# gorjanradevski/revisiting-spatial-temporal-layouts

Hardware: AMD Instinct MI355X
Metric: clips/s STLT forward (T=32, N_obj=7, d=768) (higher is better)
Workload: dtype f32; 1 GPU; cfg2: STLT forward, T=32, N=7, d=768, H=12, 4+8 layers, 174 classes; per_gpu_batch=1024, global_batch=1024, parallelism=batch-shard x1, no collective, cls_only_last_spatial=True

## Files before the change

include/stlt_hip.h:

```cpp
#ifndef STLT_HIP_H
#define STLT_HIP_H

#include <stddef.h>
#include <stdint.h>

#ifdef __cplusplus
extern "C" {
#endif

#define STLT_VERSION 110

#define STLT_EINVAL (-1)
#define STLT_EWORKSPACE (-2)

#define STLT_ACT_NONE 0
#define STLT_ACT_GELU 1
#define STLT_ACT_RELU 2

typedef void* stlt_stream_t;

int stlt_version(void);
const char* stlt_last_error(void);

typedef struct stlt_ctx stlt_ctx;
// ... 5 lines not shown
                   const float* box_w, const float* box_b, const float* score_w, const float* score_b,
                   const float* ln_w, const float* ln_b, float eps,
                   int64_t n_tokens, int64_t d, float* out, stlt_stream_t stream);

int stlt_linear_fwd(const float* x, int64_t ldx, const float* w, const float* bias,
                    float* y, int64_t ldy, int64_t M, int64_t N, int64_t K, int act, stlt_stream_t stream);

int stlt_gemm(int transA, int transB, const float* a, int64_t lda, const float* b, int64_t ldb,
              const float* r, int64_t ldr, float* c, int64_t ldc, int64_t slab_stride,
              int64_t M, int64_t N, int64_t K, int n_split, stlt_stream_t stream);
int stlt_linear_small_fwd(const float* x, int64_t ldx, const float* w, const float* bias, const float* r, int64_t ldr, float* y, int64_t ldy,
                          int64_t M, int64_t N, int64_t K, int act, int tile, stlt_stream_t stream);
int stlt_linear_small_choice(int64_t M, int64_t N, int64_t K);
int stlt_input_grad_small(const float* dy, int64_t ld_dy, const float* w, int64_t n_out, int64_t k_in, const float* r, int64_t ldr, float* dx,
                          int64_t ld_dx, int64_t M, int tile, stlt_ctx* ctx, stlt_stream_t stream);
int stlt_input_grad_small_choice(int64_t M, int64_t n_out, int64_t k_in);
int stlt_set_gemm_small_tiles(int mode);

size_t stlt_gemm_scratch_bytes(void);
int stlt_gemm_set_scratch(void* scratch, size_t bytes);
typedef struct { const float* dy; int64_t n_out; const float* x; int64_t k_in; int64_t rows; float* g_w; } stlt_wgrad_item;
int stlt_weight_grad_group(const stlt_wgrad_item* items, int n_items, stlt_stream_t stream);
int stlt_reduce_slabs(const float* slabs, int64_t stride, int n_slabs, float* dst, int64_t n, int accumulate,
                      stlt_stream_t stream);

int stlt_attn_core_fwd(const float* qkv, const uint8_t* kpm, int causal,
                       int64_t S, int64_t L, int64_t H, int64_t dh, float* ctx, stlt_stream_t stream);

int stlt_mhsa_fused_fwd(const float* x, const float* in_proj_w, const float* in_proj_b, const uint8_t* kpm, int64_t S, int64_t L,
                        int64_t H, int64_t d, float* ctx, stlt_stream_t stream);
int stlt_mhsa_fused_fwd_ex(const float* x, const float* in_proj_w, const float* in_proj_b, const uint8_t* kpm, int causal, int64_t S,
                           int64_t L, int64_t H, int64_t d, float dropout_p, uint64_t seed, uint32_t site, float* ctx, float* qkv_out,
                           stlt_stream_t stream);
int stlt_fused_mhsa_active(int64_t T, int64_t d, int64_t H);
int stlt_fused_mhsa_used(int64_t S, int64_t L, int64_t d, int64_t H, int causal);
int stlt_attn_cross_fwd(const float* q, int64_t ldq, const float* k, const float* v, int64_t ldkv, const uint8_t* kpm,
                        int causal, int64_t S, int64_t Lq, int64_t Lk, int64_t H, int64_t dh, float* ctx,
                        stlt_stream_t stream);

int stlt_attn_ragged_fwd(const float* qkv, const int32_t* seg_start, const int32_t* seg_end, int causal, int64_t M,
                         int64_t H, int64_t dh, float* ctx, stlt_stream_t stream);

int stlt_add_layernorm_fwd(const float* x, int64_t ldx, const float* res, int64_t ldres,
                           const float* ln_w, const float* ln_b, float eps,
                           int64_t M, int64_t d, float* out, int64_t ldout, stlt_stream_t stream);

int stlt_frames_embed_fwd(const float* spatial, int64_t row_stride, const int64_t* frame_types,
                          const float* pos_table, const float* type_table,
                          const float* ln_w, const float* ln_b, float eps,
                          int64_t B, int64_t T, int64_t d, float* out, stlt_stream_t stream);

int stlt_gather_last_fwd(const float* x, const int64_t* lengths, int64_t B, int64_t T, int64_t d,
                         float* out, stlt_stream_t stream);

int stlt_collate_fwd(const int64_t* categories_ragged, const float* boxes_ragged, const float* scores_ragged,
                     const int64_t* frame_types_ragged, const int64_t* frame_offsets, int64_t B, int64_t T, int64_t N,
                     int64_t cls_id, int64_t* categories, float* boxes, float* scores, int64_t* frame_types,
                     uint8_t* kpm_boxes, uint8_t* kpm_frames, stlt_stream_t stream);

typedef struct {
  int64_t src_offset;
  int32_t h, w;
  int32_t rh, rw;
  int32_t top, left;
  int32_t tab_x, ksize_x;
  int32_t tab_y, ksize_y;
// ... 308 lines not shown
```

revisiting-spatial-temporal-layouts_amd/_lib.py:

```python
from __future__ import annotations

import ctypes as C
import os

HERE = os.path.dirname(os.path.abspath(__file__))
LIB_PATH = os.environ.get("STLT_HIP_LIB") or os.path.join(HERE, "libstlt_hip.so")

K_NAMES = ("embed", "gemm", "attn_spatial", "attn_temporal", "add_layernorm", "frames_embed", "gather_last", "ln_bwd", "attn_bwd",
           "gelu", "embed_bwd", "optim", "misc", "mhsa_fused", "mhsa_fused_spatial")
FLAG_CLS_ONLY_LAST_SPATIAL = 1
FLAG_LAST_ROW_ONLY_TEMPORAL = 2
FLAG_SKIP_PADDING = 4
FLAG_TRAIN_UPPER_ONLY = 8
FLAG_TRAIN_LOWER_ONLY = 16
FLAG_TRAIN_BACKBONE = 32
ACT_NONE, ACT_GELU, ACT_RELU = 0, 1, 2

_f = C.POINTER(C.c_float)
_i64 = C.POINTER(C.c_int64)
_u8 = C.POINTER(C.c_uint8)
_vp = C.c_void_p


class OptChunk(C.Structure):
# ... 103 lines not shown
    "stlt_version": (C.c_int, []),
    "stlt_last_error": (C.c_char_p, []),
    "stlt_embed_fwd": (C.c_int, [_vp, _vp, _vp, _vp, C.c_int64, _vp, _vp, _vp, _vp, _vp, _vp, C.c_float,
                                 C.c_int64, C.c_int64, _vp, _vp]),
    "stlt_linear_fwd": (C.c_int, [_vp, C.c_int64, _vp, _vp, _vp, C.c_int64, C.c_int64, C.c_int64, C.c_int64,
                                  C.c_int, _vp]),
    "stlt_linear_small_fwd": (C.c_int, [_vp, C.c_int64, _vp, _vp, _vp, C.c_int64, _vp, C.c_int64, C.c_int64, C.c_int64, C.c_int64, C.c_int, C.c_int, _vp]),
    "stlt_linear_small_choice": (C.c_int, [C.c_int64, C.c_int64, C.c_int64]),
    "stlt_input_grad_small": (C.c_int, [_vp, C.c_int64, _vp, C.c_int64, C.c_int64, _vp, C.c_int64, _vp, C.c_int64, C.c_int64, C.c_int, _vp, _vp]),
    "stlt_input_grad_small_choice": (C.c_int, [C.c_int64, C.c_int64, C.c_int64]),
    "stlt_set_gemm_small_tiles": (C.c_int, [C.c_int]),
    "stlt_set_train_side_stream": (C.c_int, [C.c_int]),
    "stlt_get_train_side_stream": (C.c_int, []),
    "stlt_ctx_create": (C.c_int, [C.POINTER(_vp)]),
    "stlt_ctx_destroy": (C.c_int, [_vp]),
    "stlt_ctx_dw_defer": (C.c_int, [_vp, C.c_int]),
    "stlt_ctx_dw_pending": (C.c_int, [_vp]),
    "stlt_ctx_dw_flush": (C.c_int, [_vp, _vp, C.c_size_t, _vp]),
    "stlt_ctx_wt_refresh": (C.c_int, [_vp, _vp, C.c_int64, _vp]),
    "stlt_ctx_wt_clear": (C.c_int, [_vp]),
    "stlt_ctx_wt_hits": (C.c_longlong, [_vp]),
    "stlt_gemm": (C.c_int, [C.c_int, C.c_int, _vp, C.c_int64, _vp, C.c_int64, _vp, C.c_int64, _vp, C.c_int64, C.c_int64,
                            C.c_int64, C.c_int64, C.c_int64, C.c_int, _vp]),
    "stlt_weight_grad_group": (C.c_int, [_vp, C.c_int, _vp]),
    "stlt_gemm_scratch_bytes": (C.c_size_t, []),
    "stlt_gemm_set_scratch": (C.c_int, [_vp, C.c_size_t]),
    "stlt_reduce_slabs": (C.c_int, [_vp, C.c_int64, C.c_int, _vp, C.c_int64, C.c_int, _vp]),
    "stlt_attn_core_fwd": (C.c_int, [_vp, _vp, C.c_int, C.c_int64, C.c_int64, C.c_int64, C.c_int64, _vp, _vp]),
    "stlt_mhsa_fused_fwd": (C.c_int, [_vp, _vp, _vp, _vp, C.c_int64, C.c_int64, C.c_int64, C.c_int64, _vp, _vp]),
    "stlt_fused_mhsa_active": (C.c_int, [C.c_int64, C.c_int64, C.c_int64]),
    "stlt_fused_mhsa_used": (C.c_int, [C.c_int64, C.c_int64, C.c_int64, C.c_int64, C.c_int]),
    "stlt_mhsa_fused_fwd_ex": (C.c_int, [_vp, _vp, _vp, _vp, C.c_int, C.c_int64, C.c_int64, C.c_int64, C.c_int64, C.c_float, C.c_uint64, C.c_uint32,
                                         _vp, _vp, _vp]),
    "stlt_attn_cross_fwd": (C.c_int, [_vp, C.c_int64, _vp, _vp, C.c_int64, _vp, C.c_int, C.c_int64, C.c_int64, C.c_int64,
                                      C.c_int64, C.c_int64, _vp, _vp]),
    "stlt_attn_ragged_fwd": (C.c_int, [_vp, _vp, _vp, C.c_int, C.c_int64, C.c_int64, C.c_int64, _vp, _vp]),
    "stlt_add_layernorm_fwd": (C.c_int, [_vp, C.c_int64, _vp, C.c_int64, _vp, _vp, C.c_float, C.c_int64, C.c_int64,
                                         _vp, C.c_int64, _vp]),
    "stlt_frames_embed_fwd": (C.c_int, [_vp, C.c_int64, _vp, _vp, _vp, _vp, _vp, C.c_float, C.c_int64, C.c_int64,
                                        C.c_int64, _vp, _vp]),
    "stlt_gather_last_fwd": (C.c_int, [_vp, _vp, C.c_int64, C.c_int64, C.c_int64, _vp, _vp]),
    "stlt_collate_fwd": (C.c_int, [_vp, _vp, _vp, _vp, _vp, C.c_int64, C.c_int64, C.c_int64, C.c_int64, _vp, _vp, _vp, _vp,
                                   _vp, _vp, _vp]),
    "stlt_video_prep_workspace_bytes": (C.c_size_t, [C.c_int64, C.c_int64, C.c_int64]),
    "stlt_video_prep_fwd": (C.c_int, [_vp, C.c_int64, C.POINTER(VideoClip), _vp, C.c_int64, _vp, C.c_int64, C.c_int64, C.c_int64, _vp, _vp,
                                      C.c_size_t, _vp]),
    "stlt_layout_boxes_fwd": (C.c_int, [_vp, _vp, C.c_int64, _vp, _vp]),
    "stlt_layout_batch_fwd": (C.c_int, [C.POINTER(LayoutTable), _vp, _vp, C.c_int64, C.c_int64, C.c_int64, C.c_int64, _vp, _vp, _vp, _vp, _vp, _vp,
                                        _vp, _vp, _vp]),
    "stlt_frames_resize_workspace_bytes": (C.c_size_t, [C.c_int64] * 7),
    "stlt_frames_resize_fwd": (C.c_int, [_vp, C.c_int64, C.c_int64, C.c_int64, C.c_int64, C.c_int64, _vp, C.c_int64, _vp, C.c_int64, _vp, C.c_int64,
                                         C.c_int64, _vp, C.c_size_t, _vp]),
    "stlt_frames_batch_block_bytes": (C.c_size_t, [C.c_int64, C.c_int64]),
    "stlt_frames_batch_fwd": (C.c_int, [_vp, C.c_int64, _vp, C.c_int64, _vp, _vp, _vp, C.c_int64, C.c_int64, C.c_int64, _vp, _vp, _vp]),
    "stlt_workspace_bytes": (C.c_size_t, [C.c_int64, C.c_int64, C.c_int64, C.c_int64, C.c_int64]),
    "stlt_backbone_forward": (C.c_int, [C.POINTER(Params), C.POINTER(Inputs), _vp, C.c_size_t, C.c_int, _vp, _vp]),
    "stlt_forward": (C.c_int, [C.POINTER(Params), C.POINTER(Inputs), _vp, C.c_size_t, C.c_int, _vp, _vp, _vp]),
    "stlt_caf_workspace_bytes": (C.c_size_t, [C.c_int64] * 7),
    "stlt_caf_forward": (C.c_int, [C.c_void_p, C.POINTER(Inputs), _vp, _vp, C.c_size_t, _vp, _vp, _vp, _vp, _vp]),
    "stlt_caf_forward_flags": (C.c_int, [C.c_void_p, C.POINTER(Inputs), _vp, _vp, C.c_size_t, C.c_int, _vp, _vp, _vp, _vp, _vp]),
    "stlt_train_tape_bytes": (C.c_size_t, [C.c_int64] * 6),
    "stlt_train_scratch_bytes": (C.c_size_t, [C.c_int64] * 5),
    "stlt_train_forward": (C.c_int, [C.POINTER(Params), C.POINTER(Inputs), _vp, C.c_size_t, _vp, C.c_float, C.c_uint64, C.c_int, _vp]),
    "stlt_train_backward": (C.c_int, [C.POINTER(Params), C.POINTER(Params), C.POINTER(Inputs), _vp, C.c_size_t, _vp,
                                      C.c_size_t, _vp, C.c_float, C.c_uint64, C.c_int, _vp, _vp]),
    "stlt_linear_bwd_scratch_bytes": (C.c_size_t, [C.c_int64]),
# ... 98 lines not shown
```

revisiting-spatial-temporal-layouts_amd/build.py:

```python
from __future__ import annotations

import concurrent.futures
import hashlib
import os
import shutil
import subprocess
import sys

HERE = os.path.dirname(os.path.abspath(__file__))
ROOT = os.path.dirname(HERE)
CSRC = os.path.join(HERE, "csrc")
LIB = os.path.join(HERE, "libstlt_hip.so")
OBJ = os.path.join(ROOT, "build", "obj")
SOURCES = ["api.hip", "rowwise.hip", "gemm.hip", "attn.hip", "backward.hip", "train.hip", "collate.hip", "caf.hip", "ragged.hip",
           "optim.hip", "bwd_api.hip", "evalk.hip", "attn16.hip", "attn_bwd16.hip", "attn_bwdx16.hip", "wt_cache.hip", "mhsa.hip", "blocks.hip", "gemm_bf16x3.hip", "gemm16.hip", "gemm16_rb4.hip", "gemm16_rb2.hip", "attn_any.hip", "gemm_any.hip", "r3d.hip", "video.hip", "layout_data.hip", "frame_store.hip"]
BASE_FLAGS = ["-O3", "--offload-arch=gfx950", "-std=c++17", "-fPIC", "-fno-gpu-rdc"]
FILE_FLAGS = {"gemm_bf16x3.hip": ("-fno-slp-vectorize",)}


def _hipcc() -> str:
    for c in (os.environ.get("HIPCC"), shutil.which("hipcc"), "/opt/rocm/bin/hipcc"):
        if c and os.path.exists(c):
            return c
    raise RuntimeError("hipcc not found (set HIPCC=/path/to/hipcc)")


def _headers():
    return [os.path.join(CSRC, f) for f in sorted(os.listdir(CSRC)) if f.endswith(".h")] + [os.path.join(ROOT, "include", "stlt_hip.h")]


def _sources():
    missing = [s for s in SOURCES if not os.path.exists(os.path.join(CSRC, s))]
    if missing:
        raise RuntimeError(f"HIP sources missing from {CSRC}: {missing}")
    return list(SOURCES)


def needs_build() -> bool:
    if not os.path.exists(LIB):
        return True
    t = os.path.getmtime(LIB)
    deps = [os.path.join(CSRC, f) for f in os.listdir(CSRC)] + [os.path.join(ROOT, "include", "stlt_hip.h"), os.path.abspath(__file__)]
    return any(os.path.getmtime(d) > t for d in deps)


def _digest(src: str, flags) -> str:
    h = hashlib.sha1()
    for path in [src, *_headers()]:
# ... 57 lines not shown
```

revisiting-spatial-temporal-layouts_amd/csrc/api.hip:

```cpp
#include <cstdarg>
#include <cstdlib>
#include <cstdio>
#include <cstring>
#include <mutex>
#include <vector>

#include "common.h"

namespace {
thread_local char g_err[512] = "";

struct ProfRec { int kid; hipEvent_t a, b; double flops, bytes; int kernels; char note[STLT_PROF_NOTE]; };
thread_local char t_note[STLT_PROF_NOTE] = "";
thread_local double t_flops = 0.0, t_bytes = 0.0;
thread_local int t_kernels = 0;
std::mutex g_prof_mu;
bool g_prof_on = false;
std::vector<ProfRec> g_prof_recs[STLT_MAX_DEVICES];
std::vector<hipEvent_t> g_event_pool[STLT_MAX_DEVICES];
thread_local hipEvent_t g_open_start = nullptr;
thread_local int g_scope_depth = 0;
double g_gemm_flops[STLT_MAX_DEVICES] = {};

hipEvent_t get_event(int dev) {
// ... 374 lines not shown
int stlt_head(const stlt_head_params& h, const float* x, int64_t ldx, int64_t in_dim, int64_t B, int64_t d, int64_t K, float eps,
              float* h1, float* h2, float* logits, hipStream_t s) {
  TRY(launch_linear(x, ldx, h.fc1_w, h.fc1_b, h1, d, B, d, in_dim, STLT_ACT_GELU, s));
  TRY(launch_add_layernorm(h1, d, nullptr, 0, h.ln_w, h.ln_b, eps, B, d, h2, d, s));
  return launch_linear(h2, d, h.fc2_w, h.fc2_b, logits, K, B, K, d, STLT_ACT_NONE, s);
}

static int backbone_impl(const stlt_params* p, const stlt_inputs* in, void* workspace, size_t workspace_bytes,
                         int flags, float* out_btd, float* last_rows, hipStream_t s) {
  const int64_t B = in->B, T = in->T, N = in->N, d = p->d, H = p->H;
  const WsLayout w = ws_layout(B, T, N, d, p->n_classes < 0 ? 0 : p->n_classes);
  if (!workspace || workspace_bytes < w.total)
    return stlt_set_error(STLT_EWORKSPACE, "workspace %zu B < required %zu B", workspace_bytes, w.total);
  char* base = (char*)workspace;
  StltGemmScratch gemm_scratch(base + w.sk, STLT_GEMM_SCRATCH_BYTES);
  float* x = (float*)(base + w.x);
  float* x1 = (float*)(base + w.x1);
  float* qkv = (float*)(base + w.qkv);
  float* ctx = (float*)(base + w.ctx);
  float* tmp = (float*)(base + w.tmp);
  float* hh = (float*)(base + w.hh);

  const int64_t tok = B * T * N, BT = B * T;
  TRY(launch_embed(in->categories, in->boxes, in->scores, p->cat_emb, p->n_categories, p->box_w, p->box_b, p->score_w,
                   p->score_b, p->emb_ln_w, p->emb_ln_b, p->ln_eps, tok, d, x, s));
  const bool cls_only = (flags & STLT_FLAG_CLS_ONLY_LAST_SPATIAL) && p->n_spatial > 0 && N > 1;
  const int64_t full_layers = cls_only ? p->n_spatial - 1 : p->n_spatial;
  for (int64_t l = 0; l < full_layers; ++l)
    TRY(encoder_layer(p->spatial[l], d, H, x, tok, BT, N, in->kpm_boxes, nullptr, nullptr, 0, STLT_K_ATTN_SPATIAL, qkv, ctx, tmp, x1, hh, x, s));
  const float* cls_rows = x;
  int64_t cls_stride = N * d;
  if (cls_only) {
    const stlt_layer_params& lp = p->spatial[p->n_spatial - 1];
    TRY(launch_linear(x, d, lp.in_proj_w + d * d, lp.in_proj_b + d, qkv + d, 3 * d, tok, 2 * d, d, STLT_ACT_NONE, s));
    TRY(launch_linear(x, N * d, lp.in_proj_w, lp.in_proj_b, qkv, N * 3 * d, BT, d, d, STLT_ACT_NONE, s));
    TRY(launch_attn(qkv, in->kpm_boxes, 0, BT, N, H, d / H, ctx, STLT_K_ATTN_SPATIAL, s));
    TRY(encoder_tail(lp, d, ctx, N * d, x, N * d, BT, false, tmp, x1, hh, ctx, s));
    cls_rows = ctx;
    cls_stride = d;
  }
  float* tbuf = p->n_temporal > 0 ? x1 : out_btd;
  TRY(launch_frames_embed(cls_rows, cls_stride, in->frame_types, p->pos_emb, p->type_emb, p->frames_ln_w,
                          p->frames_ln_b, p->ln_eps, B, T, d, tbuf, s));
  const int64_t n_full = last_rows ? p->n_temporal - 1 : p->n_temporal;
  for (int64_t l = 0; l < n_full; ++l) {
    float* dst = (l == p->n_temporal - 1) ? out_btd : tbuf;
    TRY(encoder_layer(p->temporal[l], d, H, tbuf, BT, B, T, in->kpm_frames, nullptr, nullptr, 1, STLT_K_ATTN_TEMPORAL, qkv, ctx, tmp,
                      x, hh, dst, s));
  }
  if (last_rows) {
    const stlt_layer_params& lp = p->temporal[p->n_temporal - 1];
    float* g_ctx = x;
    float* g_res = x + (size_t)B * d;
    float* g_x1 = hh + (size_t)B * 4 * d;
    TRY(qkv_attention(lp, d, H, tbuf, BT, B, T, in->kpm_frames, nullptr, nullptr, 1, STLT_K_ATTN_TEMPORAL, qkv, ctx, s));
    TRY(launch_gather_last(ctx, in->lengths, B, T, d, g_ctx, s));
    TRY(launch_gather_last(tbuf, in->lengths, B, T, d, g_res, s));
    TRY(encoder_tail(lp, d, g_ctx, d, g_res, d, B, false, tmp, g_x1, hh, last_rows, s));
  }
  return 0;
}

static int encoder_tail_rows(const stlt_layer_params& lp, int64_t d, const float* ctx, const float* x, const int* rows, int64_t n,
                             float* g_ctx, float* g_res, float* g_x1, float* tmp, float* hh, float* out, hipStream_t s) {
  TRY(launch_gather_rows(ctx, d, rows, n, d, g_ctx, s));
  TRY(launch_gather_rows(x, d, rows, n, d, g_res, s));
  return encoder_tail(lp, d, g_ctx, d, g_res, d, n, false, tmp, g_x1, hh, out, s);
}

static int forward_ragged(const stlt_params* p, const stlt_inputs* in, void* workspace, const WsLayout& w, float* h0, float* out_btd,
                          hipStream_t s) {
  const int64_t B = in->B, T = in->T, N = in->N, d = p->d, H = p->H;
  if (d / H != 64 && (N > 1024 || T > 1024))
    return stlt_set_error(STLT_EINVAL, "skip-padding with head dim %lld (not 64) takes at most 1024 object slots / frames per segment (N=%lld, T=%lld)", (long long)(d / H), (long long)N, (long long)T);
  char* base = (char*)workspace;
  float* x = (float*)(base + w.x);
  float* x1 = (float*)(base + w.x1);
  float* qkv = (float*)(base + w.qkv);
  float* ctx = (float*)(base + w.ctx);
  float* tmp = (float*)(base + w.tmp);
  float* hh = (float*)(base + w.hh);
  const RaggedIndex ix = ragged_index_carve(base + w.ridx, B, T, N);
  TRY(launch_ragged_index(in->kpm_boxes, in->kpm_frames, in->lengths, B, T, N, ix, s));
  int64_t Ms = 0, Mf = 0;
  bool host_counts = false;
  TRY(read_ragged_counts(ix, in, true, Ms, Mf, &host_counts, s));
  TRY(launch_embed(in->categories, in->boxes, in->scores, p->cat_emb, p->n_categories, p->box_w, p->box_b, p->score_w,
                   p->score_b, p->emb_ln_w, p->emb_ln_b, p->ln_eps, Ms, d, x, s, nullptr, StltDrop{0u, 1.0f, 0ull}, ix.t_orig));
  for (int64_t l = 0; l + 1 < p->n_spatial; ++l)
    TRY(encoder_layer(p->spatial[l], d, H, x, Ms, 0, 0, nullptr, ix.t_seg_start, ix.t_seg_end, 0, STLT_K_ATTN_SPATIAL, qkv, ctx, tmp, x1, hh, x, s));
// ... 85 lines not shown
```

revisiting-spatial-temporal-layouts_amd/csrc/common.h:

```cpp
#pragma once
#include <hip/hip_runtime.h>
#include <stdint.h>
#include "stlt_hip.h"

typedef float f32x4 __attribute__((ext_vector_type(4)));
typedef float f32x2 __attribute__((ext_vector_type(2)));
typedef float f32x16 __attribute__((ext_vector_type(16)));

#define STLT_WAVE 64

int stlt_set_error(int code, const char* fmt, ...);
int stlt_check_launch(const char* what);
#define TRY(expr) do { int _e = (expr); if (_e) return _e; } while (0)
constexpr size_t stlt_align256(size_t v) { return (v + 255) / 256 * 256; }

constexpr int STLT_MAX_DEVICES = 64;
int stlt_current_device();
int stlt_device_cus();
struct StltPerDeviceOnce {
  bool done[STLT_MAX_DEVICES] = {};
  bool& flag() { return done[stlt_current_device() & (STLT_MAX_DEVICES - 1)]; }
};
struct StltPerDeviceInt {
  int v[STLT_MAX_DEVICES] = {};
// ... 212 lines not shown
bool stlt_gemm_has_scratch();
int launch_reduce_slabs(const float* slabs, int64_t stride, int n_slabs, float* dst, int64_t n, int accumulate, hipStream_t s);
struct StltReduceEntry { const float* slabs; float* dst[3]; int64_t stride, n; int n_slabs, n_dst; };
constexpr int STLT_REDUCE_DEFER_MAX = 48;
struct StltReduceDefer {
  StltReduceEntry e[STLT_REDUCE_DEFER_MAX];
  int n = 0;
  hipStream_t s = nullptr;
  float* pool = nullptr;
  size_t pool_floats = 0, used = 0;
  int err = 0;
};
void stlt_reduce_defer_set(StltReduceDefer* d);
int stlt_reduce_defer_flush(StltReduceDefer* d);
float* stlt_reduce_defer_chunk(StltReduceDefer* d, size_t floats, float* fallback, int* err);
int launch_reduce_slabs3(const float* slabs, int64_t stride, int n_slabs, float* dst0, float* dst1, float* dst2, int64_t n, int accumulate,
                         hipStream_t s);
int launch_attn(const float* qkv, const uint8_t* kpm, int causal, int64_t S, int64_t L, int64_t H, int64_t dh,
                float* ctx, int kid, hipStream_t s, StltDrop dr = StltDrop{0u, 1.0f, 0ull}, uint32_t site = 0);
int launch_attn16(const float* qkv, const uint8_t* kpm, int causal, int64_t S, int64_t L, int64_t H, float* ctx, int reverse, hipStream_t s,
                  bool* taken, StltDrop dr = StltDrop{0u, 1.0f, 0ull}, uint32_t site = 0);
int launch_attn_bwdx16(const float* q, int64_t ldq, const float* k, const float* v, int64_t ldkv, const float* dctx, const uint8_t* kpm,
                       int64_t S, int64_t Lq, int64_t Lk, int64_t H, float* dq, int64_t lddq, float* dk, float* dv, int64_t lddkv, StltDrop dr,
                       uint32_t site, hipStream_t s, bool* taken);
int launch_attn_bwd16(const float* qkv, const float* dctx, const uint8_t* kpm, int causal, int64_t S, int64_t L, int64_t H, float* dqkv,
                      StltDrop dr, uint32_t site, float* scratch, int want_colsum, int* chunks_out, hipStream_t s,
                      bool* taken);
bool stlt_mhsa_fused_takes(int64_t L, int64_t H, int64_t d, int causal);
bool stlt_mhsa_fused_pays(int64_t S, int64_t L, int64_t H, int64_t d, int causal);
bool stlt_fused_mhsa_on(int causal);
int launch_mhsa_fused(const float* x, const float* w_in, const float* b_in, const uint8_t* kpm, int64_t S, int64_t L, int64_t H,
                      int64_t d, float* ctx, hipStream_t s, int causal = 1, float* qkv_out = nullptr,
                      StltDrop dr = StltDrop{0u, 1.0f, 0ull}, uint32_t site = 0);
struct AttnBwdRagged;
int launch_attn_bwd16_ragged(const float* qkv, const float* dctx, const AttnBwdRagged& rg, int causal, int64_t H, float* dqkv, StltDrop dr,
                             uint32_t site, float* scratch, int want_colsum, int* chunks_out, hipStream_t s, bool* taken);
int launch_attn_general(const float* q, int64_t ldq, const float* k, const float* v, int64_t ldkv, const uint8_t* kpm,
                        int causal, int64_t S, int64_t Lq, int64_t Lk, int64_t H, int64_t dh, float* ctx, int kid,
                        hipStream_t s, StltDrop dr = StltDrop{0u, 1.0f, 0ull}, uint32_t site = 0);
int launch_add_layernorm(const float* x, int64_t ldx, const float* res, int64_t ldres, const float* w, const float* b,
                         float eps, int64_t M, int64_t d, float* out, int64_t ldout, hipStream_t s, StltDrop dr = StltDrop{0u, 1.0f, 0ull},
                         uint32_t site = 0, const int* drop_rows = nullptr);
int stlt_linear_add_norm(const float* x, int64_t ldx, int64_t K, const float* w, const float* b, const float* res, int64_t ldres,
                         const float* ln_w, const float* ln_b, float eps, int64_t M, int64_t d, bool fuse, float* tmp, float* out,
                         hipStream_t s);
int stlt_ffn_norm(const float* x, int64_t ldx, const float* w1, const float* b1, int act, const float* w2, const float* b2,
                  const float* ln_w, const float* ln_b, float eps, int64_t M, int64_t d, bool fuse, float* hh, float* tmp, float* out,
                  hipStream_t s);
int stlt_head(const stlt_head_params& h, const float* x, int64_t ldx, int64_t in_dim, int64_t B, int64_t d, int64_t K, float eps,
              float* h1, float* h2, float* logits, hipStream_t s);
int backbone_impl_public(const stlt_params* p, const stlt_inputs* in, void* workspace, size_t workspace_bytes, int flags,
                         float* out_btd, hipStream_t s);
size_t stlt_workspace_bytes_public(int64_t B, int64_t T, int64_t N, int64_t d, int64_t n_classes);
int launch_frames_embed(const float* spatial, int64_t row_stride, const int64_t* frame_types, const float* pos_table,
                        const float* type_table, const float* ln_w, const float* ln_b, float eps, int64_t B, int64_t T,
                        int64_t d, float* out, hipStream_t s, float* pre_out = nullptr, StltDrop dr = StltDrop{0u, 1.0f, 0ull},
                        const int* src_index = nullptr, int64_t n_rows = 0);
int launch_gather_last(const float* x, const int64_t* lengths, int64_t B, int64_t T, int64_t d, float* out,
                       hipStream_t s);

struct RaggedIndex {
  int *t_seg_start, *t_seg_end, *t_orig;
  int *f_seg_start, *f_seg_end, *f_orig, *f_cls_row;
  int *last_row;
  int *clip_tok, *clip_frm, *clip_tok_off, *clip_frm_off;
  int *f_row_of;
// ... 55 lines not shown
```

revisiting-spatial-temporal-layouts_amd/ops.py:

```python
from __future__ import annotations

import ctypes as C
import threading
from typing import Optional

import torch

from . import _lib as L


def _stream() -> int:
    return torch.cuda.current_stream().cuda_stream


def _chk(t: torch.Tensor, dtype, name: str) -> torch.Tensor:
    if not isinstance(t, torch.Tensor) or not t.is_cuda:
        raise L.StltHipError(f"{name}: expected a GPU tensor (the STLT hot path has no CPU fallback), got "
                             f"{getattr(t, 'device', type(t))}")
    if t.dtype != dtype:
        raise L.StltHipError(f"{name}: expected dtype {dtype}, got {t.dtype}")
    if not t.is_contiguous():
        raise L.StltHipError(f"{name}: tensor must be contiguous")
    return t

# ... 178 lines not shown
    L.check(lib.stlt_attn_core_bwd(_p(qkv), _p(dctx), _p(kpm), int(bool(causal)), S, Lq, num_heads, d3 // 3 // num_heads, float(dropout_p), int(seed),
                                   int(site), _p(dqkv), _p(gb), sc.data_ptr(), sc.numel(), _stream()), "stlt_attn_core_bwd")
    return (dqkv, gb) if want_bias_grad else dqkv


def mhsa_fused(x: torch.Tensor, in_proj_w: torch.Tensor, in_proj_b: torch.Tensor, kpm: torch.Tensor, num_heads: int, causal: bool = True,
               want_qkv: bool = False, dropout_p: float = 0.0, seed: int = 0, site: int = 0):
    lib = L.load()
    _chk(x, torch.float32, "x"); _chk(in_proj_w, torch.float32, "in_proj_w"); _chk(in_proj_b, torch.float32, "in_proj_b")
    kpm = _mask_u8(kpm, "kpm")
    S, Lq, d = x.shape
    ctx = torch.empty_like(x)
    if not (want_qkv or dropout_p > 0.0) and causal:
        L.check(lib.stlt_mhsa_fused_fwd(_p(x), _p(in_proj_w), _p(in_proj_b), _p(kpm), S, Lq, num_heads, d, _p(ctx), _stream()), "stlt_mhsa_fused_fwd")
        return ctx
    qkv = torch.empty(S, Lq, 3 * d, device=x.device, dtype=torch.float32) if (want_qkv or dropout_p > 0.0) else None
    L.check(lib.stlt_mhsa_fused_fwd_ex(_p(x), _p(in_proj_w), _p(in_proj_b), _p(kpm), int(bool(causal)), S, Lq, num_heads, d, float(dropout_p), int(seed),
                                       int(site), _p(ctx), _p(qkv), _stream()), "stlt_mhsa_fused_fwd_ex")
    return (ctx, qkv) if qkv is not None else ctx


def attn_core(qkv: torch.Tensor, kpm: torch.Tensor, causal: bool, num_heads: int):
    lib = L.load()
    _chk(qkv, torch.float32, "qkv")
    kpm = _mask_u8(kpm, "kpm")
    S, Lq, d3 = qkv.shape
    d = d3 // 3
    ctx = torch.empty(S, Lq, d, device=qkv.device, dtype=torch.float32)
    L.check(lib.stlt_attn_core_fwd(_p(qkv), _p(kpm), int(bool(causal)), S, Lq, num_heads, d // num_heads, _p(ctx),
                                   _stream()), "stlt_attn_core_fwd")
    return ctx


def attn_cross(q: torch.Tensor, kv: torch.Tensor, kpm_k: Optional[torch.Tensor], num_heads: int, causal: bool = False):
    lib = L.load()
    _chk(q, torch.float32, "q"); _chk(kv, torch.float32, "kv")
    S, Lq, d = q.shape
    Lk = kv.shape[1]
    if kpm_k is None:
        kpm_k = torch.zeros(S, Lk, dtype=torch.uint8, device=q.device)
    kpm_k = _mask_u8(kpm_k, "kpm")
    ctx = torch.empty(S, Lq, d, device=q.device, dtype=torch.float32)
    L.check(lib.stlt_attn_cross_fwd(_p(q), d, _p(kv), kv.data_ptr() + 4 * d, 2 * d, _p(kpm_k), int(bool(causal)), S, Lq, Lk,
                                    num_heads, d // num_heads, _p(ctx), _stream()), "stlt_attn_cross_fwd")
    return ctx


def attn_ragged(qkv: torch.Tensor, seg_lengths, heads: int, causal: bool = False) -> torch.Tensor:
    lib = L.load()
    _chk(qkv, torch.float32, "qkv")
    M, d3 = qkv.shape
    d = d3 // 3
    lens = torch.as_tensor(seg_lengths, dtype=torch.int64)
    assert int(lens.sum()) == M and bool((lens > 0).all())
    ends = torch.cumsum(lens, 0)
    starts = ends - lens
    seg_start = torch.repeat_interleave(starts, lens).to(torch.int32).to(qkv.device)
    seg_end = torch.repeat_interleave(ends, lens).to(torch.int32).to(qkv.device)
    ctx = torch.empty(M, d, device=qkv.device, dtype=torch.float32)
    L.check(lib.stlt_attn_ragged_fwd(_p(qkv), _p(seg_start), _p(seg_end), int(causal), M, heads, d // heads, _p(ctx), _stream()),
            "stlt_attn_ragged_fwd")
    return ctx


def add_layernorm(x: torch.Tensor, res: Optional[torch.Tensor], w: torch.Tensor, b: torch.Tensor, eps: float):
    lib = L.load()
# ... 570 lines not shown
```

Measured before the change: 9878 clips/s.

## Absorb key/value projections into single-query attention for the last spatial and temporal layers

Adds an absorbed attention path for layers where only one query row per sequence is needed: the last spatial layer with cls_only, and the last temporal layer's final frame. Each head's query is folded through the key weights into input space, and softmax scores are taken directly against raw token rows. The attention-weighted token sum is then projected through the value weights. This avoids computing K and V projections for every token, replacing large GEMMs with per-head small GEMMs plus a rowwise kernel. The cost is many more small kernel launches, a scratch buffer, and slightly different floating-point ordering (the key bias is dropped because softmax is invariant to it).

Measured after the change: 10150 clips/s (median of 6 runs). +2.8%, better.

```diff
diff --git a/include/stlt_hip.h b/include/stlt_hip.h
--- a/include/stlt_hip.h
+++ b/include/stlt_hip.h
@@ -61,6 +61,11 @@
 int stlt_mhsa_fused_fwd_ex(const float* x, const float* in_proj_w, const float* in_proj_b, const uint8_t* kpm, int causal, int64_t S,
                            int64_t L, int64_t H, int64_t d, float dropout_p, uint64_t seed, uint32_t site, float* ctx, float* qkv_out,
                            stlt_stream_t stream);
+
+size_t stlt_attn_absorbed_scratch_bytes(int64_t S, int64_t H, int64_t d);
+size_t stlt_attn_absorbed_scratch_bytes_min(int64_t S, int64_t H, int64_t d);
+int stlt_attn_absorbed_fwd(const float* x, const int64_t* lengths, const uint8_t* kpm, const float* in_proj_w, const float* in_proj_b, int64_t S,
+                           int64_t L, int64_t H, int64_t d, void* scratch, size_t scratch_bytes, float* ctx, stlt_stream_t stream);
 int stlt_fused_mhsa_active(int64_t T, int64_t d, int64_t H);
 int stlt_fused_mhsa_used(int64_t S, int64_t L, int64_t d, int64_t H, int causal);
 int stlt_attn_cross_fwd(const float* q, int64_t ldq, const float* k, const float* v, int64_t ldkv, const uint8_t* kpm,
diff --git a/revisiting-spatial-temporal-layouts_amd/_lib.py b/revisiting-spatial-temporal-layouts_amd/_lib.py
--- a/revisiting-spatial-temporal-layouts_amd/_lib.py
+++ b/revisiting-spatial-temporal-layouts_amd/_lib.py
@@ -159,6 +159,9 @@
     "stlt_fused_mhsa_used": (C.c_int, [C.c_int64, C.c_int64, C.c_int64, C.c_int64, C.c_int]),
     "stlt_mhsa_fused_fwd_ex": (C.c_int, [_vp, _vp, _vp, _vp, C.c_int, C.c_int64, C.c_int64, C.c_int64, C.c_int64, C.c_float, C.c_uint64, C.c_uint32,
                                          _vp, _vp, _vp]),
+    "stlt_attn_absorbed_scratch_bytes": (C.c_size_t, [C.c_int64, C.c_int64, C.c_int64]),
+    "stlt_attn_absorbed_scratch_bytes_min": (C.c_size_t, [C.c_int64, C.c_int64, C.c_int64]),
+    "stlt_attn_absorbed_fwd": (C.c_int, [_vp, _vp, _vp, _vp, _vp, C.c_int64, C.c_int64, C.c_int64, C.c_int64, _vp, C.c_size_t, _vp, _vp]),
     "stlt_attn_cross_fwd": (C.c_int, [_vp, C.c_int64, _vp, _vp, C.c_int64, _vp, C.c_int, C.c_int64, C.c_int64, C.c_int64,
                                       C.c_int64, C.c_int64, _vp, _vp]),
     "stlt_attn_ragged_fwd": (C.c_int, [_vp, _vp, _vp, C.c_int, C.c_int64, C.c_int64, C.c_int64, _vp, _vp]),
diff --git a/revisiting-spatial-temporal-layouts_amd/build.py b/revisiting-spatial-temporal-layouts_amd/build.py
--- a/revisiting-spatial-temporal-layouts_amd/build.py
+++ b/revisiting-spatial-temporal-layouts_amd/build.py
@@ -13,7 +13,7 @@
 LIB = os.path.join(HERE, "libstlt_hip.so")
 OBJ = os.path.join(ROOT, "build", "obj")
 SOURCES = ["api.hip", "rowwise.hip", "gemm.hip", "attn.hip", "backward.hip", "train.hip", "collate.hip", "caf.hip", "ragged.hip",
-           "optim.hip", "bwd_api.hip", "evalk.hip", "attn16.hip", "attn_bwd16.hip", "attn_bwdx16.hip", "wt_cache.hip", "mhsa.hip", "blocks.hip", "gemm_bf16x3.hip", "gemm16.hip", "gemm16_rb4.hip", "gemm16_rb2.hip", "attn_any.hip", "gemm_any.hip", "r3d.hip", "video.hip", "layout_data.hip", "frame_store.hip"]
+           "optim.hip", "bwd_api.hip", "evalk.hip", "attn16.hip", "attn_bwd16.hip", "attn_bwdx16.hip", "wt_cache.hip", "mhsa.hip", "blocks.hip", "gemm_bf16x3.hip", "gemm16.hip", "gemm16_rb4.hip", "gemm16_rb2.hip", "attn_any.hip", "gemm_any.hip", "r3d.hip", "video.hip", "layout_data.hip", "frame_store.hip", "absorb.hip"]
 BASE_FLAGS = ["-O3", "--offload-arch=gfx950", "-std=c++17", "-fPIC", "-fno-gpu-rdc"]
 FILE_FLAGS = {"gemm_bf16x3.hip": ("-fno-slp-vectorize",)}
 
diff --git a/revisiting-spatial-temporal-layouts_amd/csrc/absorb.hip b/revisiting-spatial-temporal-layouts_amd/csrc/absorb.hip
--- /dev/null
+++ b/revisiting-spatial-temporal-layouts_amd/csrc/absorb.hip
@@ -0,0 +1,282 @@
+#include "common.h"
+#include "wave_dpp.h"
+
+#include <stdlib.h>
+
+namespace {
+
+constexpr int ABS_LR = 8;
+constexpr int ABS_MAX_L = 64;
+constexpr int ABS_E = 64;
+
+__device__ __forceinline__ float dot4(f32x4 a, f32x4 b, float acc) {
+  acc = fmaf(a[0], b[0], acc);
+  acc = fmaf(a[1], b[1], acc);
+  acc = fmaf(a[2], b[2], acc);
+  return fmaf(a[3], b[3], acc);
+}
+
+__device__ __forceinline__ float wave_max(float v) {
+#pragma unroll
+  for (int o = 32; o > 0; o >>= 1) v = fmaxf(v, __shfl_xor(v, o, 64));
+  return v;
+}
+
+__device__ __forceinline__ int query_index(const int64_t* __restrict__ lengths, int64_t seq, int L) {
+  if (!lengths) return 0;
+  int64_t t = lengths[seq] - 1;
+  t = t < 0 ? t + L : t;
+  t = t < 0 ? 0 : (t >= L ? L - 1 : t);
+  return (int)t;
+}
+
+template <int NV>
+__global__ __launch_bounds__(256) void absorbed_resident_kernel(const float* __restrict__ x, const int64_t* __restrict__ lengths,
+                                                                const uint8_t* __restrict__ kpm, float* __restrict__ work,
+                                                                float* __restrict__ flags, int64_t S, int L, int H, int d, float scale) {
+  const int lane = threadIdx.x & 63;
+  const int64_t seq = (int64_t)blockIdx.x * 4 + (threadIdx.x >> 6);
+  if (seq >= S) return;
+  const int d4 = d >> 2;
+  const int lim = lengths ? query_index(lengths, seq, L) : L - 1;
+  const f32x4* xs = reinterpret_cast<const f32x4*>(x + seq * (int64_t)L * d);
+  f32x4 xr[ABS_LR][NV];
+  bool ok[ABS_LR];
+  bool any = false;
+#pragma unroll
+  for (int j = 0; j < ABS_LR; ++j) {
+    ok[j] = j <= lim && __builtin_amdgcn_readfirstlane((int)kpm[seq * L + (j < L ? j : 0)]) == 0;
+    any |= ok[j];
+#pragma unroll
+    for (int i = 0; i < NV; ++i) {
+      const int c = i * 64 + lane;
+      xr[j][i] = (ok[j] && c < d4) ? xs[j * d4 + c] : f32x4{0.f, 0.f, 0.f, 0.f};
+    }
+  }
+  f32x4* wq = reinterpret_cast<f32x4*>(work + seq * (int64_t)H * d);
+  f32x4 qt[NV], qn[NV];
+#pragma unroll
+  for (int i = 0; i < NV; ++i) {
+    const int c = i * 64 + lane;
+    qt[i] = c < d4 ? wq[c] : f32x4{0.f, 0.f, 0.f, 0.f};
+  }
+  for (int h = 0; h < H; ++h) {
+    if (h + 1 < H) {
+#pragma unroll
+      for (int i = 0; i < NV; ++i) {
+        const int c = i * 64 + lane;
+        qn[i] = c < d4 ? wq[(h + 1) * d4 + c] : f32x4{0.f, 0.f, 0.f, 0.f};
+      }
+    }
+    float sc[ABS_LR];
+    float m = -1e30f;
+#pragma unroll
+    for (int j = 0; j < ABS_LR; ++j) {
+      sc[j] = -1e30f;
+      if (ok[j]) {
+        float a = 0.f;
+#pragma unroll
+        for (int i = 0; i < NV; ++i) a = dot4(qt[i], xr[j][i], a);
+        sc[j] = wave_sum_dpp(a) * scale;
+      }
+      m = fmaxf(m, sc[j]);
+    }
+    float sum = 0.f;
+#pragma unroll
+    for (int j = 0; j < ABS_LR; ++j) {
+      sc[j] = ok[j] ? __expf(sc[j] - m) : 0.f;
+      sum += sc[j];
+    }
+    const float inv = sum > 0.f ? 1.0f / sum : 0.f;
+    f32x4 xb[NV];
+#pragma unroll
+    for (int i = 0; i < NV; ++i) xb[i] = f32x4{0.f, 0.f, 0.f, 0.f};
+#pragma unroll
+    for (int j = 0; j < ABS_LR; ++j) {
+      const float p = sc[j] * inv;
+#pragma unroll
+      for (int i = 0; i < NV; ++i) xb[i] += p * xr[j][i];
+    }
+#pragma unroll
+    for (int i = 0; i < NV; ++i) {
+      const int c = i * 64 + lane;
+      if (c < d4) wq[h * d4 + c] = xb[i];
+      qt[i] = qn[i];
+    }
+  }
+  if (lane == 0) flags[seq] = any ? 1.f : 0.f;
+}
+
+template <int NV>
+__global__ __launch_bounds__(256) void absorbed_streamed_kernel(const float* __restrict__ x, const int64_t* __restrict__ lengths,
+                                                                const uint8_t* __restrict__ kpm, float* __restrict__ work,
+                                                                float* __restrict__ flags, int64_t S, int L, int H, int d, float scale) {
+  const int lane = threadIdx.x & 63;
+  const int64_t w = (int64_t)blockIdx.x * 4 + (threadIdx.x >> 6);
+  if (w >= S * H) return;
+  const int64_t seq = w / H;
+  const int h = (int)(w - seq * H);
+  const int d4 = d >> 2;
+  const int lim = lengths ? query_index(lengths, seq, L) : L - 1;
+  const bool valid = lane <= lim && kpm[seq * L + lane] == 0;
+  const unsigned long long vm = __ballot(valid);
+  const f32x4* xs = reinterpret_cast<const f32x4*>(x + seq * (int64_t)L * d);
+  f32x4* wq = reinterpret_cast<f32x4*>(work + (seq * H + h) * (int64_t)d);
+  f32x4 qt[NV];
+#pragma unroll
+  for (int i = 0; i < NV; ++i) {
+    const int c = i * 64 + lane;
+    qt[i] = c < d4 ? wq[c] : f32x4{0.f, 0.f, 0.f, 0.f};
+  }
+  float sc = -1e30f;
+  for (int j = 0; j <= lim; ++j) {
+    if (!((vm >> j) & 1ull)) continue;
+    float a = 0.f;
+#pragma unroll
+    for (int i = 0; i < NV; ++i) {
+      const int c = i * 64 + lane;
+      if (c < d4) a = dot4(qt[i], xs[j * d4 + c], a);
+    }
+    a = wave_sum_dpp(a);
+    if (lane == j) sc = a * scale;
+  }
+  const float m = wave_max(sc);
+  float p = valid ? __expf(sc - m) : 0.f;
+  const float sum = wave_sum_dpp(p);
+  p *= sum > 0.f ? 1.0f / sum : 0.f;
+  f32x4 xb[NV];
+#pragma unroll
+  for (int i = 0; i < NV; ++i) xb[i] = f32x4{0.f, 0.f, 0.f, 0.f};
+  for (int j = 0; j <= lim; ++j) {
+    if (!((vm >> j) & 1ull)) continue;
+    const float pj = __builtin_bit_cast(float, __builtin_amdgcn_readlane(__builtin_bit_cast(int, p), j));
+#pragma unroll
+    for (int i = 0; i < NV; ++i) {
+      const int c = i * 64 + lane;
+      if (c < d4) xb[i] += pj * xs[j * d4 + c];
+    }
+  }
+#pragma unroll
+  for (int i = 0; i < NV; ++i) {
+    const int c = i * 64 + lane;
+    if (c < d4) wq[c] = xb[i];
+  }
+  if (h == 0 && lane == 0) flags[seq] = vm != 0ull ? 1.f : 0.f;
+}
+
+__global__ __launch_bounds__(256) void absorbed_zero_masked_kernel(const float* __restrict__ flags, float* __restrict__ ctx, int64_t S, int d) {
+  const int64_t seq = (int64_t)blockIdx.x * 4 + (threadIdx.x >> 6);
+  if (seq >= S || flags[seq] != 0.f) return;
+  for (int c = (threadIdx.x & 63) * 4; c < d; c += 256) *reinterpret_cast<f32x4*>(ctx + seq * d + c) = f32x4{0.f, 0.f, 0.f, 0.f};
+}
+
+inline int nv_of(int64_t d) { return (int)((d / 4 + 63) / 64); }
+inline bool resident_shape(int64_t L, int64_t d) { return L <= ABS_LR && nv_of(d) <= 4; }
+
+int launch_rowwise(const float* x, const int64_t* lengths, const uint8_t* kpm, float* work, float* flags, int64_t S, int64_t L, int64_t H, int64_t d,
+                   hipStream_t s) {
+  const float scale = 0.125f;
+  const bool resident = resident_shape(L, d);
+  StltProfScope ps(STLT_K_MISC, s);
+  stlt_prof_note("absorbed_attn(%s) S=%lld L=%lld H=%lld d=%lld", resident ? "resident" : "streamed", (long long)S, (long long)L, (long long)H, (long long)d);
+  stlt_prof_add_bytes(4.0 * (double)S * ((double)L * d + 2.0 * H * d));
+  stlt_prof_note_flops(4.0 * (double)S * H * L * d);
+  const int nv = nv_of(d);
+#define ABS_LAUNCH(KERNEL, GRID, NVMAX)                                                                                                         \
+  switch (nv) {                                                                                                                           \
+    case 1: hipLaunchKernelGGL(KERNEL<1>, dim3((unsigned)(GRID)), dim3(256), 0, s, x, lengths, kpm, work, flags, S, (int)L, (int)H, (int)d, scale); break; \
+    case 2: hipLaunchKernelGGL(KERNEL<2>, dim3((unsigned)(GRID)), dim3(256), 0, s, x, lengths, kpm, work, flags, S, (int)L, (int)H, (int)d, scale); break; \
+    case 3: hipLaunchKernelGGL(KERNEL<3>, dim3((unsigned)(GRID)), dim3(256), 0, s, x, lengths, kpm, work, flags, S, (int)L, (int)H, (int)d, scale); break; \
+    case 4: hipLaunchKernelGGL(KERNEL<4>, dim3((unsigned)(GRID)), dim3(256), 0, s, x, lengths, kpm, work, flags, S, (int)L, (int)H, (int)d, scale); break; \
+    default: hipLaunchKernelGGL(KERNEL<NVMAX>, dim3((unsigned)(GRID)), dim3(256), 0, s, x, lengths, kpm, work, flags, S, (int)L, (int)H, (int)d, scale); break; \
+  }
+  if (resident) {
+    if (nv > 4) return stlt_set_error(STLT_EINVAL, "attn_absorbed: no resident kernel for d=%lld", (long long)d);
+    ABS_LAUNCH(absorbed_resident_kernel, (S + 3) / 4, 4)
+    return stlt_check_launch("absorbed_resident_kernel");
+  }
+  ABS_LAUNCH(absorbed_streamed_kernel, (S * H + 3) / 4, 8)
+#undef ABS_LAUNCH
+  return stlt_check_launch("absorbed_streamed_kernel");
+}
+
+}
+
+bool stlt_absorb_kv_on() {
+  static const bool on = [] { const char* e = getenv("STLT_ABSORB_KV"); return e ? atoi(e) != 0 : true; }();
+  return on;
+}
+
+bool stlt_absorb_kv_takes(int64_t S, int64_t L, int64_t H, int64_t d, size_t work_floats) {
+  return S > 0 && L >= 1 && L <= ABS_MAX_L && H >= 1 && H <= 32 && d == ABS_E * H && work_floats >= (size_t)(H * d + 1) && S * H <= 0x7fffff00LL;
+}
+bool stlt_absorb_kv_pays(int temporal, int64_t S, int64_t L, int64_t d) {
+  static const int64_t min_tokens = [] { const char* e = getenv("STLT_ABSORB_KV_MIN_TOKENS"); return e ? (int64_t)atoll(e) : (int64_t)32768; }();
+  return (temporal || resident_shape(L, d)) && S * L >= min_tokens;
+}
+
+int stlt_attn_absorbed(const float* x, int64_t L, const float* qrows, int64_t ldqr, const int64_t* lengths, const uint8_t* kpm, const float* w_in,
+                       const float* b_in, int64_t S, int64_t H, int64_t d, float* q, float* work, size_t work_floats, float* ctx, hipStream_t s) {
+  if (!x || !qrows || !kpm || !w_in || !b_in || !q || !work || !ctx) return stlt_set_error(STLT_EINVAL, "attn_absorbed: null pointer");
+  if (!stlt_absorb_kv_takes(S, L, H, d, work_floats))
+    return stlt_set_error(STLT_EINVAL, "attn_absorbed: S=%lld L=%lld H=%lld d=%lld: needs 64-channel heads (at most 32), at most %d rows per sequence and scratch for one sequence",
+                          (long long)S, (long long)L, (long long)H, (long long)d, ABS_MAX_L);
+  const int64_t e = ABS_E, per_seq = H * d + 1;
+  const int64_t cap = (int64_t)(work_floats / (size_t)per_seq);
+  TRY(launch_linear(qrows, ldqr, w_in, b_in, q, d, S, d, d, STLT_ACT_NONE, s));
+  for (int64_t s0 = 0; s0 < S; s0 += cap) {
+    const int64_t n = S - s0 < cap ? S - s0 : cap;
+    float* flags = work + n * H * d;
+    for (int64_t h = 0; h < H; ++h)
+      TRY(launch_gemm(0, 1, q + s0 * d + h * e, d, w_in + (d + h * e) * d, d, nullptr, nullptr, 0, work + h * d, H * d, 0, n, d, e, 1, STLT_ACT_NONE, s));
+    TRY(launch_rowwise(x + s0 * L * d, lengths ? lengths + s0 : nullptr, kpm + s0 * L, work, flags, n, L, H, d, s));
+    for (int64_t h = 0; h < H; ++h)
+      TRY(launch_linear(work + h * d, H * d, w_in + (2 * d + h * e) * d, b_in + 2 * d + h * e, ctx + s0 * d + h * e, d, n, e, d, STLT_ACT_NONE, s));
+    {
+      StltProfScope ps(STLT_K_MISC, s);
+      stlt_prof_note("absorbed_attn(zero masked) S=%lld d=%lld", (long long)n, (long long)d);
+      stlt_prof_add_bytes(4.0 * (double)n);
+      hipLaunchKernelGGL(absorbed_zero_masked_kernel, dim3((unsigned)((n + 3) / 4)), dim3(256), 0, s, flags, ctx + s0 * d, n, (int)d);
+      TRY(stlt_check_launch("absorbed_zero_masked_kernel"));
+    }
+  }
+  return 0;
+}
+
+extern "C" {
+
+size_t stlt_attn_absorbed_scratch_bytes(int64_t S, int64_t H, int64_t d) {
+  if (S <= 0 || H <= 0 || d <= 0) return 0;
+  return stlt_align256((size_t)S * d * sizeof(float)) * 2 + stlt_align256(((size_t)S * (H * d + 1)) * sizeof(float));
+}
+size_t stlt_attn_absorbed_scratch_bytes_min(int64_t S, int64_t H, int64_t d) {
+  if (S <= 0 || H <= 0 || d <= 0) return 0;
+  return stlt_align256((size_t)S * d * sizeof(float)) * 2 + (size_t)(H * d + 1) * sizeof(float);
+}
+
+int stlt_attn_absorbed_fwd(const float* x, const int64_t* lengths, const uint8_t* kpm, const float* in_proj_w, const float* in_proj_b, int64_t S,
+                           int64_t L, int64_t H, int64_t d, void* scratch, size_t scratch_bytes, float* ctx, stlt_stream_t stream) {
+  if (!x || !scratch) return stlt_set_error(STLT_EINVAL, "stlt_attn_absorbed_fwd: null pointer");
+  if (S <= 0 || L <= 0 || H <= 0 || H > 32 || d != ABS_E * H || L > ABS_MAX_L)
+    return stlt_set_error(STLT_EINVAL, "stlt_attn_absorbed_fwd: S=%lld L=%lld H=%lld d=%lld: needs d == 64*H, H <= 32, 1 <= L <= %d", (long long)S, (long long)L,
+                          (long long)H, (long long)d, ABS_MAX_L);
+  if (scratch_bytes < stlt_attn_absorbed_scratch_bytes_min(S, H, d))
+    return stlt_set_error(STLT_EINVAL, "stlt_attn_absorbed_fwd: scratch %zu B < stlt_attn_absorbed_scratch_bytes_min", scratch_bytes);
+  hipStream_t s = (hipStream_t)stream;
+  const size_t rows = stlt_align256((size_t)S * d * sizeof(float));
+  float* g = (float*)scratch;
+  float* q = (float*)((char*)scratch + rows);
+  float* work = (float*)((char*)scratch + 2 * rows);
+  const float* qrows = x;
+  int64_t ldqr = L * d;
+  if (lengths) {
+    TRY(launch_gather_last(x, lengths, S, L, d, g, s));
+    qrows = g;
+    ldqr = d;
+  }
+  size_t work_floats = (scratch_bytes - 2 * rows) / sizeof(float);
+  if (work_floats > (size_t)S * (H * d + 1)) work_floats = (size_t)S * (H * d + 1);
+  return stlt_attn_absorbed(x, L, qrows, ldqr, lengths, kpm, in_proj_w, in_proj_b, S, H, d, q, work, work_floats, ctx, s);
+}
+
+}
diff --git a/revisiting-spatial-temporal-layouts_amd/csrc/api.hip b/revisiting-spatial-temporal-layouts_amd/csrc/api.hip
--- a/revisiting-spatial-temporal-layouts_amd/csrc/api.hip
+++ b/revisiting-spatial-temporal-layouts_amd/csrc/api.hip
@@ -430,10 +430,15 @@
   int64_t cls_stride = N * d;
   if (cls_only) {
     const stlt_layer_params& lp = p->spatial[p->n_spatial - 1];
-    TRY(launch_linear(x, d, lp.in_proj_w + d * d, lp.in_proj_b + d, qkv + d, 3 * d, tok, 2 * d, d, STLT_ACT_NONE, s));
-    TRY(launch_linear(x, N * d, lp.in_proj_w, lp.in_proj_b, qkv, N * 3 * d, BT, d, d, STLT_ACT_NONE, s));
-    TRY(launch_attn(qkv, in->kpm_boxes, 0, BT, N, H, d / H, ctx, STLT_K_ATTN_SPATIAL, s));
-    TRY(encoder_tail(lp, d, ctx, N * d, x, N * d, BT, false, tmp, x1, hh, ctx, s));
+    if (stlt_absorb_kv_on() && stlt_absorb_kv_pays(0, BT, N, d) && stlt_absorb_kv_takes(BT, N, H, d, (size_t)tok * 4 * d)) {
+      TRY(stlt_attn_absorbed(x, N, x, N * d, nullptr, in->kpm_boxes, lp.in_proj_w, lp.in_proj_b, BT, H, d, tmp, hh, (size_t)tok * 4 * d, ctx, s));
+      TRY(encoder_tail(lp, d, ctx, d, x, N * d, BT, false, tmp, x1, hh, ctx, s));
+    } else {
+      TRY(launch_linear(x, d, lp.in_proj_w + d * d, lp.in_proj_b + d, qkv + d, 3 * d, tok, 2 * d, d, STLT_ACT_NONE, s));
+      TRY(launch_linear(x, N * d, lp.in_proj_w, lp.in_proj_b, qkv, N * 3 * d, BT, d, d, STLT_ACT_NONE, s));
+      TRY(launch_attn(qkv, in->kpm_boxes, 0, BT, N, H, d / H, ctx, STLT_K_ATTN_SPATIAL, s));
+      TRY(encoder_tail(lp, d, ctx, N * d, x, N * d, BT, false, tmp, x1, hh, ctx, s));
+    }
     cls_rows = ctx;
     cls_stride = d;
   }
@@ -451,9 +456,14 @@
     float* g_ctx = x;
     float* g_res = x + (size_t)B * d;
     float* g_x1 = hh + (size_t)B * 4 * d;
-    TRY(qkv_attention(lp, d, H, tbuf, BT, B, T, in->kpm_frames, nullptr, nullptr, 1, STLT_K_ATTN_TEMPORAL, qkv, ctx, s));
-    TRY(launch_gather_last(ctx, in->lengths, B, T, d, g_ctx, s));
-    TRY(launch_gather_last(tbuf, in->lengths, B, T, d, g_res, s));
+    if (stlt_absorb_kv_on() && stlt_absorb_kv_pays(1, B, T, d) && stlt_absorb_kv_takes(B, T, H, d, (size_t)tok * 4 * d)) {
+      TRY(launch_gather_last(tbuf, in->lengths, B, T, d, g_res, s));
+      TRY(stlt_attn_absorbed(tbuf, T, g_res, d, in->lengths, in->kpm_frames, lp.in_proj_w, lp.in_proj_b, B, H, d, tmp, hh, (size_t)tok * 4 * d, g_ctx, s));
+    } else {
+      TRY(qkv_attention(lp, d, H, tbuf, BT, B, T, in->kpm_frames, nullptr, nullptr, 1, STLT_K_ATTN_TEMPORAL, qkv, ctx, s));
+      TRY(launch_gather_last(ctx, in->lengths, B, T, d, g_ctx, s));
+      TRY(launch_gather_last(tbuf, in->lengths, B, T, d, g_res, s));
+    }
     TRY(encoder_tail(lp, d, g_ctx, d, g_res, d, B, false, tmp, g_x1, hh, last_rows, s));
   }
   return 0;
diff --git a/revisiting-spatial-temporal-layouts_amd/csrc/common.h b/revisiting-spatial-temporal-layouts_amd/csrc/common.h
--- a/revisiting-spatial-temporal-layouts_amd/csrc/common.h
+++ b/revisiting-spatial-temporal-layouts_amd/csrc/common.h
@@ -268,6 +268,11 @@
 int launch_mhsa_fused(const float* x, const float* w_in, const float* b_in, const uint8_t* kpm, int64_t S, int64_t L, int64_t H,
                       int64_t d, float* ctx, hipStream_t s, int causal = 1, float* qkv_out = nullptr,
                       StltDrop dr = StltDrop{0u, 1.0f, 0ull}, uint32_t site = 0);
+bool stlt_absorb_kv_on();
+bool stlt_absorb_kv_takes(int64_t S, int64_t L, int64_t H, int64_t d, size_t work_floats);
+bool stlt_absorb_kv_pays(int temporal, int64_t S, int64_t L, int64_t d);
+int stlt_attn_absorbed(const float* x, int64_t L, const float* qrows, int64_t ldqr, const int64_t* lengths, const uint8_t* kpm, const float* w_in,
+                       const float* b_in, int64_t S, int64_t H, int64_t d, float* q, float* work, size_t work_floats, float* ctx, hipStream_t s);
 struct AttnBwdRagged;
 int launch_attn_bwd16_ragged(const float* qkv, const float* dctx, const AttnBwdRagged& rg, int causal, int64_t H, float* dqkv, StltDrop dr,
                              uint32_t site, float* scratch, int want_colsum, int* chunks_out, hipStream_t s, bool* taken);
diff --git a/revisiting-spatial-temporal-layouts_amd/ops.py b/revisiting-spatial-temporal-layouts_amd/ops.py
--- a/revisiting-spatial-temporal-layouts_amd/ops.py
+++ b/revisiting-spatial-temporal-layouts_amd/ops.py
@@ -234,6 +234,24 @@
     return ctx
 
 
+def attn_absorbed(x: torch.Tensor, in_proj_w: torch.Tensor, in_proj_b: torch.Tensor, kpm: torch.Tensor, num_heads: int,
+                  lengths: Optional[torch.Tensor] = None, chunk_sequences: Optional[int] = None):
+    lib = L.load()
+    _chk(x, torch.float32, "x"); _chk(in_proj_w, torch.float32, "in_proj_w"); _chk(in_proj_b, torch.float32, "in_proj_b")
+    kpm = _mask_u8(kpm, "kpm")
+    if lengths is not None:
+        _chk(lengths, torch.int64, "lengths")
+    S, Lq, d = x.shape
+    ctx = torch.empty(S, d, device=x.device, dtype=torch.float32)
+    nbytes = int(lib.stlt_attn_absorbed_scratch_bytes(S, num_heads, d))
+    if chunk_sequences is not None:
+        nbytes = min(nbytes, int(lib.stlt_attn_absorbed_scratch_bytes_min(S, num_heads, d)) + (int(chunk_sequences) - 1) * (num_heads * d + 1) * 4)
+    sc = torch.empty(max(nbytes, 4) // 4, device=x.device, dtype=torch.float32)
+    L.check(lib.stlt_attn_absorbed_fwd(_p(x), _p(lengths), _p(kpm), _p(in_proj_w), _p(in_proj_b), S, Lq, num_heads, d, sc.data_ptr(), nbytes, _p(ctx),
+                                       _stream()), "stlt_attn_absorbed_fwd")
+    return ctx
+
+
 def attn_cross(q: torch.Tensor, kv: torch.Tensor, kpm_k: Optional[torch.Tensor], num_heads: int, causal: bool = False):
     lib = L.load()
     _chk(q, torch.float32, "q"); _chk(kv, torch.float32, "kv")
```
